# kan-bayashi/ParallelWaveGAN

Hardware: AMD Instinct MI355X
Metric: HiFi-GAN V1 22.05 kHz generator inference RTF^-1 (audio samples/s) (higher is better)
Workload: dtype f32; 1 GPU; HiFi-GAN V1 generator fwd, LJSpeech 22.05 kHz, B16 x 800 mel frames per GPU, fp32, random init; global_batch=16, parallelism=replicas x1

## Files before the change

### include/pwg_kernels.h

```cpp
#ifndef PWG_KERNELS_H_
#define PWG_KERNELS_H_

#include <stddef.h>
#include <stdint.h>

#ifdef __cplusplus
extern "C" {
#endif

typedef enum pwg_status {
  PWG_OK = 0,
  PWG_ERR_BAD_SHAPE = -1,
  PWG_ERR_UNSUPPORTED = -2,
  PWG_ERR_LAUNCH = -3,
  PWG_ERR_NULL = -4,
  PWG_ERR_WORKSPACE = -5
} pwg_status;

const char* pwg_last_error(void);
int pwg_abi_version(void);
int pwg_target_arch(void);

int pwg_prof_enable(int on);
int pwg_prof_reset(void);
// ... 64 lines not shown
int pwg_conv1d_backward_weight(const pwg_conv1d_desc* d, const float* x, const float* dy, float* dw,
                               float* db, float* workspace, size_t workspace_floats, void* stream);

size_t pwg_conv1d_backward_weight_wn_workspace_floats(const pwg_conv1d_desc* d);
int pwg_conv1d_backward_weight_wn(const pwg_conv1d_desc* d, const float* x, const float* dy, const float* v,
                                  const float* g, float* dv, float* dg, float* db, float* workspace,
                                  size_t workspace_floats, void* stream);

int pwg_conv1d_num_tile_configs(void);
int pwg_conv1d_forward_cfg(const pwg_conv1d_desc* d, const float* x, const float* w_packed,
                           const float* bias, const float* add1, const float* add2, float* y,
                           int32_t tile_config, int32_t use_dma, void* stream);

int pwg_conv1d_bf16_supported(const pwg_conv1d_desc* d);
size_t pwg_conv1d_bf16_packed_weight_bytes(const pwg_conv1d_desc* d);
int pwg_conv1d_bf16_pack_weight(const pwg_conv1d_desc* d, const float* w, const float* scale, void* w_packed,
                                void* stream);
int pwg_conv1d_bf16_forward(const pwg_conv1d_desc* d, const float* x, const void* w_packed, const float* bias,
                            const float* add1, const float* add2, float* y, float* workspace, size_t workspace_floats,
                            void* stream);
int pwg_conv1d_bf16_forward_cfg(const pwg_conv1d_desc* d, const float* x, const void* w_packed, const float* bias,
                                const float* add1, const float* add2, float* y, int32_t mfma_shape, void* stream);

int pwg_conv1d_split_supported(const pwg_conv1d_desc* d);
size_t pwg_conv1d_split_packed_weight_bytes(const pwg_conv1d_desc* d);
int pwg_conv1d_split_pack_weight(const pwg_conv1d_desc* d, const float* w, const float* scale, void* w_packed,
                                 void* stream);
int pwg_conv1d_split_forward(const pwg_conv1d_desc* d, const float* x, const void* w_packed, const float* bias,
                             const float* add1, const float* add2, float* y, float* workspace, size_t workspace_floats,
                             void* stream);
int pwg_conv1d_split_forward_cfg(const pwg_conv1d_desc* d, const float* x, const void* w_packed, const float* bias,
                                 const float* add1, const float* add2, float* y, int32_t mfma_shape, int32_t tile_mode,
                                 void* stream);

int pwg_convtr1d_split_supported(const pwg_conv1d_desc* d);
size_t pwg_convtr1d_split_packed_weight_bytes(const pwg_conv1d_desc* d);
int pwg_convtr1d_split_pack_weight(const pwg_conv1d_desc* d, const float* w, const float* scale, void* w_packed,
                                   void* stream);
int pwg_convtr1d_split_forward(const pwg_conv1d_desc* d, const float* x, const void* w_packed, const float* bias,
                               const float* add1, const float* add2, float* y, float* workspace,
                               size_t workspace_floats, void* stream);
int pwg_convtr1d_split_forward_cfg(const pwg_conv1d_desc* d, const float* x, const void* w_packed, const float* bias,
                                   const float* add1, const float* add2, float* y, int32_t mfma_shape,
                                   int32_t tile_mode, void* stream);

int pwg_conv1d_stream_supported(const pwg_conv1d_desc* d);
size_t pwg_conv1d_stream_hist_floats(const pwg_conv1d_desc* d);
int pwg_conv1d_stream_forward(const pwg_conv1d_desc* d, const float* x, const float* hist_in, float* hist_out,
                              const float* w_packed, const float* bias, const float* add1, const float* add2, float* y,
                              void* stream);

int pwg_conv1d_stream_bf16_supported(const pwg_conv1d_desc* d);
int pwg_conv1d_stream_bf16_forward(const pwg_conv1d_desc* d, const float* x, const float* hist_in, float* hist_out,
                                   const void* w_packed_bf16, const float* bias, const float* add1,
                                   const float* add2, float* y, void* stream);

int pwg_conv1d_stream_delayed_supported(const pwg_conv1d_desc* d, int32_t delay1, int32_t delay2);
int pwg_conv1d_stream_delayed_forward(const pwg_conv1d_desc* d, const float* x, const float* hist_in, float* hist_out,
                                      const float* w_packed, const float* bias, const float* add1,
                                      const float* add1_hist_in, float* add1_hist_out, int32_t delay1, const float* add2,
                                      const float* add2_hist_in, float* add2_hist_out, int32_t delay2, int32_t valid_lo,
                                      int32_t valid_hi, float* y, void* stream);

int pwg_conv1d_stream_bf16_delayed_supported(const pwg_conv1d_desc* d, int32_t delay1, int32_t delay2);
int pwg_conv1d_stream_bf16_delayed_forward(const pwg_conv1d_desc* d, const float* x, const float* hist_in,
                                           float* hist_out, const void* w_packed_bf16, const float* bias,
// ... 333 lines not shown
```

### parallelwavegan_amd/_lib.py

```python
import ctypes
import os

_HERE = os.path.dirname(os.path.abspath(__file__))
LIB_PATH = os.environ.get("PWG_KERNEL_LIB") or os.path.join(_HERE, "libpwgkernels.so")

PWG_ACT_NONE, PWG_ACT_LEAKY_RELU, PWG_ACT_TANH, PWG_ACT_RELU = 0, 1, 2, 3
PWG_PAD_ZERO, PWG_PAD_REFLECT, PWG_PAD_REPLICATE = 0, 1, 2
ABI_VERSION = 15
SPECTRAL_NORM_SCRATCH_FLOATS = 257


class ConvDesc(ctypes.Structure):

    _fields_ = [
        ("batch", ctypes.c_int32),
        ("c_in", ctypes.c_int32),
        ("c_out", ctypes.c_int32),
        ("t_in", ctypes.c_int32),
        ("t_out", ctypes.c_int32),
        ("width", ctypes.c_int32),
        ("kernel", ctypes.c_int32),
        ("stride", ctypes.c_int32),
        ("dilation", ctypes.c_int32),
        ("pad_left", ctypes.c_int32),
# ... 76 lines not shown
_i64 = ctypes.c_int64
_f32 = ctypes.c_float

SIGNATURES = {
    "pwg_last_error": (ctypes.c_char_p, []),
    "pwg_abi_version": (ctypes.c_int, []),
    "pwg_target_arch": (ctypes.c_int, []),
    "pwg_debug_poison_lds": (ctypes.c_int, [ctypes.c_int]),
    "pwg_set_concurrency_hint": (ctypes.c_float, [ctypes.c_float]),
    "pwg_prof_enable": (ctypes.c_int, [ctypes.c_int]),
    "pwg_prof_reset": (ctypes.c_int, []),
    "pwg_prof_num_kernels": (ctypes.c_int, []),
    "pwg_prof_get": (ctypes.c_int, [_i32, ctypes.c_char_p, ctypes.c_size_t, ctypes.POINTER(ctypes.c_double),
                                    ctypes.POINTER(ctypes.c_int64), ctypes.POINTER(ctypes.c_double),
                                    ctypes.POINTER(ctypes.c_double)]),
    "pwg_conv1d_packed_weight_floats": (ctypes.c_size_t, [ctypes.POINTER(ConvDesc)]),
    "pwg_conv1d_pack_weight": (ctypes.c_int, [ctypes.POINTER(ConvDesc), _vp, _vp, _vp, _vp]),
    "pwg_conv1d_forward_workspace_floats": (ctypes.c_size_t, [ctypes.POINTER(ConvDesc)]),
    "pwg_conv1d_forward": (ctypes.c_int, [ctypes.POINTER(ConvDesc), _vp, _vp, _vp, _vp, _vp, _vp, _vp, ctypes.c_size_t,
                                          _vp]),
    "pwg_conv1d_bf16_supported": (ctypes.c_int, [ctypes.POINTER(ConvDesc)]),
    "pwg_conv1d_bf16_packed_weight_bytes": (ctypes.c_size_t, [ctypes.POINTER(ConvDesc)]),
    "pwg_conv1d_bf16_pack_weight": (ctypes.c_int, [ctypes.POINTER(ConvDesc), _vp, _vp, _vp, _vp]),
    "pwg_conv1d_bf16_forward": (ctypes.c_int, [ctypes.POINTER(ConvDesc), _vp, _vp, _vp, _vp, _vp, _vp, _vp, ctypes.c_size_t,
                                               _vp]),
    "pwg_conv1d_bf16_forward_cfg": (ctypes.c_int, [ctypes.POINTER(ConvDesc), _vp, _vp, _vp, _vp, _vp, _vp, _i32, _vp]),
    "pwg_conv1d_split_supported": (ctypes.c_int, [ctypes.POINTER(ConvDesc)]),
    "pwg_conv1d_split_packed_weight_bytes": (ctypes.c_size_t, [ctypes.POINTER(ConvDesc)]),
    "pwg_conv1d_split_pack_weight": (ctypes.c_int, [ctypes.POINTER(ConvDesc), _vp, _vp, _vp, _vp]),
    "pwg_conv1d_split_forward": (ctypes.c_int, [ctypes.POINTER(ConvDesc), _vp, _vp, _vp, _vp, _vp, _vp, _vp,
                                                ctypes.c_size_t, _vp]),
    "pwg_conv1d_split_forward_cfg": (ctypes.c_int, [ctypes.POINTER(ConvDesc), _vp, _vp, _vp, _vp, _vp, _vp, _i32, _i32,
                                                    _vp]),
    "pwg_convtr1d_split_supported": (ctypes.c_int, [ctypes.POINTER(ConvDesc)]),
    "pwg_convtr1d_split_packed_weight_bytes": (ctypes.c_size_t, [ctypes.POINTER(ConvDesc)]),
    "pwg_convtr1d_split_pack_weight": (ctypes.c_int, [ctypes.POINTER(ConvDesc), _vp, _vp, _vp, _vp]),
    "pwg_convtr1d_split_forward": (ctypes.c_int, [ctypes.POINTER(ConvDesc), _vp, _vp, _vp, _vp, _vp, _vp, _vp,
                                                  ctypes.c_size_t, _vp]),
    "pwg_convtr1d_split_forward_cfg": (ctypes.c_int, [ctypes.POINTER(ConvDesc), _vp, _vp, _vp, _vp, _vp, _vp, _i32, _i32,
                                                      _vp]),
    "pwg_conv1d_stream_supported": (ctypes.c_int, [ctypes.POINTER(ConvDesc)]),
    "pwg_conv1d_stream_hist_floats": (ctypes.c_size_t, [ctypes.POINTER(ConvDesc)]),
    "pwg_conv1d_stream_forward": (ctypes.c_int, [ctypes.POINTER(ConvDesc), _vp, _vp, _vp, _vp, _vp, _vp, _vp, _vp, _vp]),
    "pwg_conv1d_stream_bf16_supported": (ctypes.c_int, [ctypes.POINTER(ConvDesc)]),
    "pwg_conv1d_stream_bf16_forward": (ctypes.c_int, [ctypes.POINTER(ConvDesc), _vp, _vp, _vp, _vp, _vp, _vp, _vp, _vp,
                                                      _vp]),
    "pwg_conv1d_stream_delayed_supported": (ctypes.c_int, [ctypes.POINTER(ConvDesc), _i32, _i32]),
    "pwg_conv1d_stream_delayed_forward": (ctypes.c_int, [ctypes.POINTER(ConvDesc), _vp, _vp, _vp, _vp, _vp, _vp, _vp, _vp,
                                                         _i32, _vp, _vp, _vp, _i32, _i32, _i32, _vp, _vp]),
    "pwg_conv1d_stream_bf16_delayed_supported": (ctypes.c_int, [ctypes.POINTER(ConvDesc), _i32, _i32]),
    "pwg_conv1d_stream_bf16_delayed_forward": (ctypes.c_int, [ctypes.POINTER(ConvDesc), _vp, _vp, _vp, _vp, _vp, _vp, _vp,
                                                              _vp, _i32, _vp, _vp, _vp, _i32, _i32, _i32, _vp, _vp]),
    "pwg_conv1d_stream_slots_forward": (ctypes.c_int, [ctypes.POINTER(ConvDesc), _vp, _vp, _vp, _vp, _vp, _vp, _vp, _vp,
                                                       _i32, _vp, _vp, _vp, _i32, _vp, _i32, _i32, _vp, _vp]),
    "pwg_conv1d_stream_slots_forward_bf16": (ctypes.c_int, [ctypes.POINTER(ConvDesc), _vp, _vp, _vp, _vp, _vp, _vp, _vp,
                                                            _vp, _i32, _vp, _vp, _vp, _i32, _vp, _i32, _i32, _vp, _vp]),
    "pwg_conv1d_stream_mirrored_supported": (ctypes.c_int, [ctypes.POINTER(ConvDesc)]),
    "pwg_conv1d_stream_mirrored_forward": (ctypes.c_int, [ctypes.POINTER(ConvDesc), _vp, _vp, _vp, _vp, _vp, _vp, _i32,
                                                          _i32, _i32, _i32, _vp]),
    "pwg_conv1d_packed_weight_bwd_floats": (ctypes.c_size_t, [ctypes.POINTER(ConvDesc)]),
    "pwg_conv1d_pack_weight_bwd": (ctypes.c_int, [ctypes.POINTER(ConvDesc), _vp, _vp, _vp, _vp]),
    "pwg_weight_bank_table_bytes": (ctypes.c_size_t, [_i32]),
    "pwg_weight_bank_build": (ctypes.c_int, [ctypes.POINTER(BankItem), _i32, _vp, ctypes.c_size_t,
                                             ctypes.POINTER(ctypes.c_int32)]),
    "pwg_weight_bank_prepare": (ctypes.c_int, [_vp, ctypes.POINTER(ctypes.c_int32), _i32, _vp]),
    "pwg_conv1d_backward_data_workspace_floats": (ctypes.c_size_t, [ctypes.POINTER(ConvDesc)]),
# ... 158 lines not shown
```

### parallelwavegan_amd/csrc/conv1d_split.hip

```cpp
#include "mfma_conv.h"

namespace pwg {
namespace {

constexpr int PARTS = 3;

struct SplitArgs : MfmaConvArgs {
  int plane;
  long part_stride;
  float pre_mul;
  unsigned pre_mask;
  int wide_out;
};

static int split_geometry(const pwg_conv1d_desc* d, MfmaConvGeom* g) {
  return mfma_conv_geometry("conv1d_split", PARTS, false, d, g);
}

__device__ __forceinline__ float pre_activate(float v, float mul, unsigned mask) {
  const float n = __uint_as_float(__float_as_uint(v * mul) & mask);
  return v > 0.f ? v : n;
}

template <int NT, bool CHECKED>
// ... 93 lines not shown
      for (int k = 0; k < NB; ++k) v[k] *= a.out_mul;
    }
    if (a.out_div != 1.0f) {
#pragma unroll
      for (int k = 0; k < NB; ++k) v[k] = v[k] / a.out_div;
    }
    if (a.post_act == PWG_ACT_LEAKY_RELU) {
#pragma unroll
      for (int k = 0; k < NB; ++k)
#pragma unroll
        for (int e = 0; e < 4; ++e) v[k][e] = v[k][e] > 0.f ? v[k][e] : v[k][e] * a.post_slope;
    } else if (a.post_act == PWG_ACT_RELU) {
#pragma unroll
      for (int k = 0; k < NB; ++k)
#pragma unroll
        for (int e = 0; e < 4; ++e) v[k][e] = v[k][e] > 0.f ? v[k][e] : 0.f;
    } else if (a.post_act == PWG_ACT_TANH) {
#pragma unroll
      for (int k = 0; k < NB; ++k) {
#pragma unroll
        for (int e = 0; e < 4; ++e) v[k][e] = tanhf(v[k][e]);
        __builtin_amdgcn_sched_barrier(0);
      }
    }
#pragma unroll
    for (int k = 0; k < NB; ++k) {
      if (WIDE) {
        if (FULL || (m < a.m && q[k] < a.nq)) *reinterpret_cast<f32x4*>(a.y + row + q[k]) = v[k];
      } else {
#pragma unroll
        for (int e = 0; e < 4; ++e)
          if (m < a.m && q[k] + e < a.nq) a.y[row + q[k] + e] = v[k][e];
      }
    }
  }
}

template <int TILE, int WM, int WN, int WAVES_M, bool VEC>
__global__ __launch_bounds__(256, WM * WN == 4 ? (TILE == 16 ? 3 : 2) : (WM * WN == 2 ? 3 : 4)) void
conv1d_split_mfma_kernel(SplitArgs a) {
  constexpr int HL = 64 / TILE;
  constexpr int KSTEPS = KC / (8 * HL);
  constexpr int TM = WM * 32 / TILE, TN = WN * 32 / TILE;
  constexpr int NREG = TILE * TILE / 64;
  constexpr int WAVES_N = 4 / WAVES_M;
  constexpr int MT = WAVES_M * WM * 32, NT = WAVES_N * WN * 32;
  typedef typename Mfma<TILE>::acc_t acc_t;

  extern __shared__ __attribute__((aligned(16))) unsigned char smem[];
  __bf16* xs = reinterpret_cast<__bf16*>(smem);

  const MfmaConvTile c = mfma_conv_tile<TILE, MT, NT, WAVES_M, VEC>(a);
  const float* __restrict__ xb = c.xb;

  acc_t acc[TM][TN];
#pragma unroll
  for (int mi = 0; mi < TM; ++mi)
#pragma unroll
    for (int ni = 0; ni < TN; ++ni)
#pragma unroll
      for (int i = 0; i < NREG; ++i) acc[mi][ni][i] = 0.f;

  for (int chunk = 0; chunk < a.cin_chunks; ++chunk) {
    if (chunk) __syncthreads();
    if (VEC) {
      const int ngroups = (c.wcols + 3) >> 2, c_left = a.c_in - chunk * KC;
// ... 19 lines not shown
            f[j] = 0.f;
            if (tin && c_base + j < a.c_in) f[j] = src[(size_t)j * a.t_in];
          }
        }
#pragma unroll
        for (int j = 0; j < 8; ++j) f[j] = pre_activate(f[j], a.pre_mul, a.pre_mask);
        split3_store<8>(f, xs + col * kConvRow + c.wave * 8, a.plane);
      }
    }
    __syncthreads();
    for (int tap = 0; tap < a.taps; ++tap) {
#pragma unroll
      for (int ks = 0; ks < KSTEPS; ++ks) {
        const int oct = ks * HL + c.h;
        const bf16x8* __restrict__ wp =
            image_rows(a.w, a.cin_chunks, a.m_pad, tap, chunk, oct) + c.m0 + c.wave_m * (WM * 32) + c.r;
        split_step<TILE, TM, TN, kConvRow, true>(wp, a.part_stride, xs, c.sh + c.wave_n * (WN * 32) + c.r + tap * a.dil,
                                                 oct * 8, a.plane, acc);
      }
    }
  }

  const size_t out_base = (size_t)c.b * a.c_out * a.t_out;
  const int row0 = c.m0 + c.wave_m * (WM * 32) + c.r, col0 = c.q0 + c.wave_n * (WN * 32) + 4 * c.h;
  const bool full = c.m0 + MT <= a.m && c.q0 + NT <= a.nq;
  if (!a.wide_out)
    split_epilogue<TILE, TM, TN, false, false>(a, acc, row0, col0, out_base);
  else if (full)
    split_epilogue<TILE, TM, TN, true, true>(a, acc, row0, col0, out_base);
  else
    split_epilogue<TILE, TM, TN, true, false>(a, acc, row0, col0, out_base);
}

template <bool VEC>
struct Family {
  template <int TILE, int WM, int WN, int WAVES_M>
  struct K {
    static constexpr auto fn = conv1d_split_mfma_kernel<TILE, WM, WN, WAVES_M, VEC>;
  };
};

static void split_fill_args(SplitArgs* a, const pwg_conv1d_desc* d, const MfmaConvGeom& g, const MfmaConvPlan& p,
                            const float* x, const void* w_packed, const float* bias, const float* add1, const float* add2,
                            float* y) {
  mfma_conv_fill_args(a, d, g, x, w_packed, bias, add1, add2, y);
  a->plane = p.plane;
  a->part_stride = image_elems(g) / 8;
  a->pre_mul = d->pre_act == PWG_ACT_LEAKY_RELU ? d->pre_slope : (d->pre_act == PWG_ACT_RELU ? 0.0f : 1.0f);
  a->pre_mask = d->pre_act == PWG_ACT_RELU ? 0u : ~0u;
  a->wide_out = d->t_out % 4 == 0 && ((reinterpret_cast<uintptr_t>(y) | reinterpret_cast<uintptr_t>(add1) |
                                       reinterpret_cast<uintptr_t>(add2)) & 15u) == 0;
}

static int split_forward(const pwg_conv1d_desc* d, const float* x, const void* w_packed, const float* bias,
                         const float* add1, const float* add2, float* y, int mfma_shape, int tile_mode,
                         hipStream_t stream) {
  MfmaConvGeom g;
  int rc = split_geometry(d, &g);
  if (rc == PWG_OK) rc = mfma_conv_check_forward("conv1d_split", d, x, w_packed, y, mfma_shape, tile_mode);
  if (rc != PWG_OK) return rc;
  const MfmaConvPlan p = mfma_conv_plan(d, g, PARTS, tile_mode, x, add1, add2);
  SplitArgs a;
  split_fill_args(&a, d, g, p, x, w_packed, bias, add1, add2, y);
  maybe_poison_lds(stream);
  ProfScope prof(stream, "conv1d_split_mfma_kernel", p.flops, p.bytes);
  if (p.vec)
    mfma_conv_launch<Family<true>::K>(p, mfma_shape, a, stream);
  else
    mfma_conv_launch<Family<false>::K>(p, mfma_shape, a, stream);
  PWG_CHECK_LAUNCH("conv1d_split");
  return PWG_OK;
}

struct ConvtrArgs : SplitArgs {
  int phases, out_off;
};

static int convtr_geometry(const pwg_conv1d_desc* d, MfmaConvGeom* g) {
  PWG_REQUIRE(d != nullptr, PWG_ERR_NULL, "convtr1d_split: NULL descriptor");
  PWG_REQUIRE(d->transposed, PWG_ERR_UNSUPPORTED,
              "convtr1d_split: not a transposed convolution (a stride-1 Conv1d runs on conv1d_split)");
  return mfma_conv_geometry("convtr1d_split", PARTS, true, d, g);
}

template <int NT, bool VEC>
__device__ __forceinline__ void stage_chunk(const SplitArgs& a, const MfmaConvTile& c, int chunk, __bf16* xs) {
  if (VEC) {
    const int ngroups = (c.wcols + 3) >> 2, c_left = a.c_in - chunk * KC;
    const float* __restrict__ xc = c.xb + (size_t)chunk * KC * a.t_in;
    if (c.base >= 0 && c.base + 4 * ngroups <= a.t_in && c_left >= KC)
      stage_window_vec<NT, false>(a, xc, c_left, c.base, ngroups, xs, c.tid);
    else
      stage_window_vec<NT, true>(a, xc, c_left, c.base, ngroups, xs, c.tid);
  } else {
    const int c_base = chunk * KC + c.wave * 8;
    const bool interior = c.base >= 0 && c.base + c.wcols <= a.t_in && c_base + 8 <= a.c_in;
    for (int col = c.lane; col < c.wcols; col += 64) {
      const int t = c.base + col;
      const float* __restrict__ src = c.xb + (size_t)c_base * a.t_in + t;
      float f[8];
      if (interior) {
#pragma unroll
        for (int j = 0; j < 8; ++j) f[j] = src[(size_t)j * a.t_in];
      } else {
        const bool tin = t >= 0 && t < a.t_in;
#pragma unroll
        for (int j = 0; j < 8; ++j) {
          f[j] = 0.f;
          if (tin && c_base + j < a.c_in) f[j] = src[(size_t)j * a.t_in];
        }
      }
#pragma unroll
      for (int j = 0; j < 8; ++j) f[j] = pre_activate(f[j], a.pre_mul, a.pre_mask);
      split3_store<8>(f, xs + col * kConvRow + c.wave * 8, a.plane);
    }
  }
}

template <int N>
__device__ __forceinline__ void convtr_finish(float out_mul, float out_div, int post_act, float post_slope, f32x4 (&v)[N],
                                              const f32x4& bias, bool has_bias, bool has1, bool has2,
                                              const f32x4 (&t1)[N], const f32x4 (&t2)[N]) {
  if (has_bias) {
#pragma unroll
    for (int k = 0; k < N; ++k) v[k] += bias;
  }
  if (has1) {
#pragma unroll
    for (int k = 0; k < N; ++k) v[k] += t1[k];
  }
  if (has2) {
#pragma unroll
    for (int k = 0; k < N; ++k) v[k] += t2[k];
  }
  if (out_mul != 1.0f) {
#pragma unroll
    for (int k = 0; k < N; ++k) v[k] *= out_mul;
  }
  if (out_div != 1.0f) {
#pragma unroll
    for (int k = 0; k < N; ++k) v[k] = v[k] / out_div;
  }
  if (post_act == PWG_ACT_LEAKY_RELU) {
#pragma unroll
    for (int k = 0; k < N; ++k)
#pragma unroll
      for (int e = 0; e < 4; ++e) v[k][e] = v[k][e] > 0.f ? v[k][e] : v[k][e] * post_slope;
  } else if (post_act == PWG_ACT_RELU) {
#pragma unroll
// ... 174 lines not shown

}
}

using namespace pwg;

extern "C" int pwg_conv1d_split_supported(const pwg_conv1d_desc* d) {
  MfmaConvGeom g;
  return split_geometry(d, &g) == PWG_OK ? 1 : 0;
}

extern "C" size_t pwg_conv1d_split_packed_weight_bytes(const pwg_conv1d_desc* d) {
  MfmaConvGeom g;
  if (split_geometry(d, &g) != PWG_OK) return 0;
  return (size_t)PARTS * image_elems(g) * sizeof(__bf16);
}

extern "C" int pwg_conv1d_split_pack_weight(const pwg_conv1d_desc* d, const float* w, const float* scale, void* w_packed,
                                            void* stream) {
  MfmaConvGeom g;
  int rc = split_geometry(d, &g);
  if (rc != PWG_OK) return rc;
  PWG_REQUIRE(w && w_packed, PWG_ERR_NULL, "conv1d_split_pack_weight: NULL pointer");
  mfma_conv_pack<PARTS>(d, g, w, scale, w_packed, (hipStream_t)stream);
  PWG_CHECK_LAUNCH("conv1d_split_pack_weight");
  return PWG_OK;
}

extern "C" int pwg_conv1d_split_forward(const pwg_conv1d_desc* d, const float* x, const void* w_packed, const float* bias,
                                        const float* add1, const float* add2, float* y, float* workspace,
                                        size_t workspace_floats, void* stream) {
  (void)workspace;
  (void)workspace_floats;
  return split_forward(d, x, w_packed, bias, add1, add2, y, kDefaultMfmaShape, 0, (hipStream_t)stream);
}

extern "C" int pwg_conv1d_split_forward_cfg(const pwg_conv1d_desc* d, const float* x, const void* w_packed,
                                            const float* bias, const float* add1, const float* add2, float* y,
                                            int32_t mfma_shape, int32_t tile_mode, void* stream) {
  return split_forward(d, x, w_packed, bias, add1, add2, y, mfma_shape, tile_mode, (hipStream_t)stream);
}

extern "C" int pwg_convtr1d_split_supported(const pwg_conv1d_desc* d) {
  MfmaConvGeom g;
  return convtr_geometry(d, &g) == PWG_OK ? 1 : 0;
}

extern "C" size_t pwg_convtr1d_split_packed_weight_bytes(const pwg_conv1d_desc* d) {
  MfmaConvGeom g;
  if (convtr_geometry(d, &g) != PWG_OK) return 0;
  return (size_t)PARTS * image_elems(g) * sizeof(__bf16);
}

extern "C" int pwg_convtr1d_split_pack_weight(const pwg_conv1d_desc* d, const float* w, const float* scale, void* w_packed,
                                              void* stream) {
  MfmaConvGeom g;
  int rc = convtr_geometry(d, &g);
  if (rc != PWG_OK) return rc;
  PWG_REQUIRE(w && w_packed, PWG_ERR_NULL, "convtr1d_split_pack_weight: NULL pointer");
  mfma_conv_pack<PARTS>(d, g, w, scale, w_packed, (hipStream_t)stream);
  PWG_CHECK_LAUNCH("convtr1d_split_pack_weight");
  return PWG_OK;
}

extern "C" int pwg_convtr1d_split_forward(const pwg_conv1d_desc* d, const float* x, const void* w_packed, const float* bias,
                                          const float* add1, const float* add2, float* y, float* workspace,
                                          size_t workspace_floats, void* stream) {
  (void)workspace;
  (void)workspace_floats;
  return convtr_forward(d, x, w_packed, bias, add1, add2, y, kDefaultMfmaShape, 0, (hipStream_t)stream);
}

extern "C" int pwg_convtr1d_split_forward_cfg(const pwg_conv1d_desc* d, const float* x, const void* w_packed,
// ... 5 lines not shown
```

### parallelwavegan_amd/csrc/resunit_split.hip

```cpp
#include "mfma_conv.h"

#include <stdlib.h>

namespace pwg {
namespace {

constexpr size_t kRuSplitMaxLds = 80 * 1024;

struct RuSplitArgs {
  const float* x;
  const bf16x8* w1;
  const float* b1;
  const bf16x8* w2;
  const float* b2;
  const float* add2;
  float* y;
  int T, k, d1;
  int bn_out;
  int hla;
  int sh;
  int p2;
  int rows;
  int plane;
  long part_stride;
  float slope1, slope2, out_div;
};

template <int C>
struct RuSplitCfg {
  static constexpr int MB = C / KC;
  static constexpr int WAVES_N = 4 / MB;
  static constexpr int H = WAVES_N * 64;
  static constexpr int ROW = C + 8;
  static constexpr int OCTS = C / 8;
  static constexpr int CHUNKS = image_chunks(C), M_PAD = image_m_pad(C);
};

template <int C, bool CHECKED>
__device__ __forceinline__ void ru_stage_window(const RuSplitArgs& a, const float* __restrict__ xb, int base, __bf16* xs,
                                                int tid) {
  constexpr int OCTS = RuSplitCfg<C>::OCTS, ROW = RuSplitCfg<C>::ROW;
  const int nitems = (a.rows >> 2) * OCTS;
  f32x4 st[2][8];
#pragma unroll
  for (int it = 0; it < 2; ++it) {
    const int idx = tid + it * 256, oct = idx % OCTS, grp = idx / OCTS;
    const int t = base + grp * 4;
    const float* __restrict__ src = xb + (size_t)(oct * 8) * a.T + t;
    const bool in = idx < nitems && (!CHECKED || (t >= 0 && t < a.T));
#pragma unroll
    for (int j = 0; j < 8; ++j) {
      f32x4 v = {0.f, 0.f, 0.f, 0.f};
      if (in) v = *reinterpret_cast<const f32x4*>(src + (size_t)j * a.T);
      st[it][j] = v;
    }
  }
#pragma unroll
  for (int it = 0; it < 2; ++it) {
    const int idx = tid + it * 256, oct = idx % OCTS, grp = idx / OCTS;
    if (idx < nitems) {
#pragma unroll
      for (int e = 0; e < 4; ++e) {
        float v[8];
#pragma unroll
        for (int j = 0; j < 8; ++j) {
          const float s = st[it][j][e];
          v[j] = s > 0.f ? s : s * a.slope1;
        }
        split3_store<8>(v, xs + (grp * 4 + e) * ROW + oct * 8, a.plane);
        __builtin_amdgcn_sched_barrier(0);
      }
    }
  }
}

template <int C, int TILE>
__device__ __forceinline__ void ru_request(bf16x8 (&wf)[3], const bf16x8* __restrict__ w, long part_stride, unsigned wrow,
                                           int h) {
  using Cfg = RuSplitCfg<C>;
  split_step_request(wf, w, part_stride, wrow + split_step_rows<TILE>(Cfg::CHUNKS, Cfg::M_PAD, SplitStepId{0, 0, 0}, h));
}
template <int C, int TILE, bool XFIRST>
__device__ __forceinline__ void ru_contract(bf16x8 (&wf)[3], const bf16x8* __restrict__ w, long part_stride, unsigned wrow,
                                            const __bf16* bl, int plane, int tap_step, int taps, int h,
                                            typename Mfma<TILE>::acc_t (&acc)[32 / TILE][64 / TILE]) {
  using Cfg = RuSplitCfg<C>;
  constexpr int HL = 64 / TILE, KSTEPS = KC / (8 * HL), TM = 32 / TILE, TN = 64 / TILE;
  SplitStepId step{0, 0, 0};
#pragma unroll 1
  for (int s = 0; s < Cfg::CHUNKS * taps * KSTEPS; ++s) {
    const SplitStepId next = split_step_successor(step, Cfg::CHUNKS, taps, KSTEPS);
    split_step_streamed<TILE, TM, TN, Cfg::ROW, XFIRST>(
        wf, w, part_stride, wrow + split_step_rows<TILE>(Cfg::CHUNKS, Cfg::M_PAD, step, h),
        wrow + split_step_rows<TILE>(Cfg::CHUNKS, Cfg::M_PAD, next, h), bl, step.tap * tap_step,
        step.chunk * KC + split_step_off<TILE>(step, h), plane, acc);
    step = next;
  }
}

template <int C, int TILE>
__global__ __launch_bounds__(256, 2) void resunit_split_kernel(RuSplitArgs a) {
  using Cfg = RuSplitCfg<C>;
  constexpr int WAVES_N = Cfg::WAVES_N, ROW = Cfg::ROW, H = Cfg::H;
  constexpr int HL = 64 / TILE, TM = 32 / TILE, TN = 64 / TILE, NREG = TILE * TILE / 64, NG = NREG / 4;
  typedef typename Mfma<TILE>::acc_t acc_t;
  extern __shared__ __attribute__((aligned(16))) unsigned char smem[];
  __bf16* xs = reinterpret_cast<__bf16*>(smem);

  const int tid = threadIdx.x, lane = tid & 63;
  const int wave = __builtin_amdgcn_readfirstlane(tid >> 6);
  const int wave_m = wave / WAVES_N, wave_n = wave % WAVES_N;
  const int r = lane & (TILE - 1), h = lane / TILE;
  const int b = blockIdx.y;
  const int t0 = blockIdx.x * a.bn_out;
  const int base = t0 - a.hla;
  const int T = a.T;
  const bool pair = a.w2 != nullptr;
  const float* __restrict__ xb = a.x + (size_t)b * C * T;

  const unsigned wrow = wave_m * 32 + r;
  bf16x8 wf[3];
  ru_request<C, TILE>(wf, a.w1, a.part_stride, wrow, h);

  if (base >= 0 && base + a.rows <= T)
    ru_stage_window<C, false>(a, xb, base, xs, tid);
  else
    ru_stage_window<C, true>(a, xb, base, xs, tid);

  acc_t acc[TM][TN];
#pragma unroll
  for (int mi = 0; mi < TM; ++mi)
#pragma unroll
    for (int ni = 0; ni < TN; ++ni)
#pragma unroll
      for (int i = 0; i < NREG; ++i) acc[mi][ni][i] = 0.f;
  __syncthreads();

  if (pair) {
    ru_contract<C, TILE, false>(wf, a.w1, a.part_stride, wrow, xs + (wave_n * 64 + r + a.sh) * ROW, a.plane, a.d1, a.k,
                                h, acc);
    ru_request<C, TILE>(wf, a.w2, a.part_stride, wrow, h);
    __syncthreads();
    const bool has_b1 = a.b1 != nullptr;
#pragma unroll
    for (int mi = 0; mi < TM; ++mi)
#pragma unroll
      for (int g = 0; g < NG; ++g) {
        const int c = wave_m * 32 + mi * TILE + 4 * h + 4 * HL * g;
        f32x4 bias = {0.f, 0.f, 0.f, 0.f};
        if (has_b1) {
#pragma unroll
          for (int e = 0; e < 4; ++e) bias[e] = a.b1[c + e];
        }
#pragma unroll
        for (int ni = 0; ni < TN; ++ni) {
          const int m = wave_n * 64 + ni * TILE + r;
          const int th = t0 - a.p2 + m;
          const bool inside = th >= 0 && th < T;
          float v[4];
#pragma unroll
          for (int e = 0; e < 4; ++e) {
            v[e] = acc[mi][ni][4 * g + e];
            if (has_b1) v[e] += bias[e];
            v[e] = v[e] > 0.f ? v[e] : v[e] * a.slope2;
            v[e] = inside ? v[e] : 0.f;
            acc[mi][ni][4 * g + e] = 0.f;
          }
          split3_store<4>(v, xs + m * ROW + c, a.plane);
        }
      }
    for (int i = tid; i < (a.k - 1) * Cfg::OCTS; i += 256) {
      bf16x8 z;
#pragma unroll
      for (int j = 0; j < 8; ++j) z[j] = (__bf16)0.f;
      __bf16* dst = xs + (H + i / Cfg::OCTS) * ROW + (i % Cfg::OCTS) * 8;
      *reinterpret_cast<bf16x8*>(dst) = z;
      *reinterpret_cast<bf16x8*>(dst + a.plane) = z;
      *reinterpret_cast<bf16x8*>(dst + 2 * a.plane) = z;
    }
    __syncthreads();
    ru_contract<C, TILE, true>(wf, a.w2, a.part_stride, wrow, xs + (wave_n * 64 + r) * ROW, a.plane, 1, a.k, h,
                               acc);
  } else {
    ru_contract<C, TILE, true>(wf, a.w1, a.part_stride, wrow, xs + (wave_n * 64 + r + a.sh) * ROW, a.plane, a.d1, a.k,
                               h, acc);
  }

  constexpr int NV = TN * NG;
  const float* __restrict__ bias_p = pair ? a.b2 : a.b1;
  const bool has_bias = bias_p != nullptr, has2 = a.add2 != nullptr;
#pragma unroll
  for (int mi = 0; mi < TM; ++mi) {
    const int c = wave_m * 32 + mi * TILE + r;
    const size_t row = ((size_t)b * C + c) * T;
    int t[NV];
    bool ok[NV];
#pragma unroll
    for (int n = 0; n < NV; ++n) {
      const int slot = wave_n * 64 + (n / NG) * TILE + 4 * h + 4 * HL * (n % NG);
      ok[n] = slot < a.bn_out && t0 + slot < T;
      t[n] = ok[n] ? t0 + slot : t0;
    }
    f32x4 t1[NV], t2[NV], v[NV];
    float bias = 0.f;
    if (has_bias) bias = bias_p[c];
#pragma unroll
    for (int n = 0; n < NV; ++n) t1[n] = *reinterpret_cast<const f32x4*>(a.x + row + t[n]);
    if (has2) {
#pragma unroll
      for (int n = 0; n < NV; ++n) t2[n] = *reinterpret_cast<const f32x4*>(a.add2 + row + t[n]);
    }
#pragma unroll
    for (int n = 0; n < NV; ++n)
#pragma unroll
      for (int e = 0; e < 4; ++e) v[n][e] = acc[mi][n / NG][(n % NG) * 4 + e];
    if (has_bias) {
#pragma unroll
      for (int n = 0; n < NV; ++n) v[n] += bias;
    }
#pragma unroll
    for (int n = 0; n < NV; ++n) v[n] += t1[n];
    if (has2) {
#pragma unroll
      for (int n = 0; n < NV; ++n) v[n] += t2[n];
    }
    if (a.out_div != 1.0f) {
#pragma unroll
      for (int n = 0; n < NV; ++n) v[n] = v[n] / a.out_div;
    }
#pragma unroll
    for (int n = 0; n < NV; ++n)
      if (ok[n]) *reinterpret_cast<f32x4*>(a.y + row + t[n]) = v[n];
  }
}

struct RuSplitGeom {
  int hla, sh, p2, bn_out, rows, tiles;
  size_t lds;
};

static int ru_split_geometry(const pwg_resunit_desc* d, RuSplitGeom* g) {
  PWG_REQUIRE(d != nullptr, PWG_ERR_NULL, "resunit_split: NULL descriptor");
  const int C = d->channels;
  PWG_REQUIRE(C == 32 || C == 64, PWG_ERR_UNSUPPORTED, "resunit_split: channels = %d (only 32 and 64)", C);
// ... 102 lines not shown
```

### parallelwavegan_amd/ops.py

```python
import ctypes

import torch

from . import _lib
from ._lib import ConvDesc, ResUnitDesc, WaveNetDesc

ACT = {None: _lib.PWG_ACT_NONE, "none": _lib.PWG_ACT_NONE, "leaky_relu": _lib.PWG_ACT_LEAKY_RELU,
       "tanh": _lib.PWG_ACT_TANH, "relu": _lib.PWG_ACT_RELU}
PAD = {"zero": _lib.PWG_PAD_ZERO, "reflect": _lib.PWG_PAD_REFLECT, "replicate": _lib.PWG_PAD_REPLICATE}


PARAM_EPOCH = [0]


def bump_param_epoch():
    PARAM_EPOCH[0] += 1


def cache_epoch():
    return PARAM_EPOCH[0]


def param_epoch(p):
    return getattr(p, "_pwg_epoch", 0)
# ... 132 lines not shown
    if out is None:
        out = torch.empty((desc.batch, desc.c_out, desc.t_out * desc.width), device=x.device, dtype=torch.float32)
    assert x.numel() == desc.batch * desc.c_in * desc.t_in * desc.width, (tuple(x.shape), desc.batch, desc.c_in, desc.t_in)
    assert out.numel() == desc.batch * desc.c_out * desc.t_out * desc.width
    ws, ws_n = _workspace(_lib.lib().pwg_conv1d_forward_workspace_floats(ctypes.byref(desc)), x.device)
    _lib.check(_lib.lib().pwg_conv1d_forward(ctypes.byref(desc), _ptr(x), _ptr(w_packed), _ptr(bias), _ptr(add1),
                                             _ptr(add2), _ptr(out), _ptr(ws), ws_n, _stream()), "conv1d_forward")
    return out


def conv1d_bf16_supported(desc):
    return bool(_lib.lib().pwg_conv1d_bf16_supported(ctypes.byref(desc)))


def _zero_padded(desc):
    if desc.pad_mode == PAD["zero"]:
        return desc
    desc = ConvDesc.from_buffer_copy(desc)
    desc.pad_mode = PAD["zero"]
    return desc


def _pack_weight_mfma(kind, desc, w, scale, op="conv1d"):
    _require_device(w, scale)
    n = getattr(_lib.lib(), f"pwg_{op}_{kind}_packed_weight_bytes")(ctypes.byref(desc))
    if n == 0:
        _lib.check(-1, f"{op}_{kind}_packed_weight_bytes")
    out = torch.empty(n, device=w.device, dtype=torch.uint8)
    pack = getattr(_lib.lib(), f"pwg_{op}_{kind}_pack_weight")
    _lib.check(pack(ctypes.byref(desc), _ptr(w), _ptr(scale), _ptr(out), _stream()), f"{op}_{kind}_pack_weight")
    return out


def _conv1d_forward_mfma(kind, desc, image_desc, x, w_packed, bias, add1, add2, out, cfg, op="conv1d"):
    name = f"{op}_forward_{kind}"
    _require_device(x, bias, add1, add2, out)
    if not w_packed.is_cuda or w_packed.dtype != torch.uint8:
        raise RuntimeError(f"{name}: w_packed must be the device image of pack_weight_{kind}")
    if out is None:
        out = torch.empty((desc.batch, desc.c_out, desc.t_out), device=x.device, dtype=torch.float32)
    assert x.numel() == desc.batch * desc.c_in * desc.t_in, (tuple(x.shape), desc.batch, desc.c_in, desc.t_in)
    assert out.numel() == desc.batch * desc.c_out * desc.t_out
    image_bytes = getattr(_lib.lib(), f"pwg_{op}_{kind}_packed_weight_bytes")(ctypes.byref(image_desc))
    if image_bytes == 0:
        _lib.check(-1, f"{op}_{kind}_packed_weight_bytes")
    assert w_packed.numel() == image_bytes, f"{name}: w_packed is not this layer's {kind} image"
    for t in (add1, add2):
        assert t is None or t.numel() == out.numel()
    args = (ctypes.byref(desc), _ptr(x), _ptr(w_packed), _ptr(bias), _ptr(add1), _ptr(add2), _ptr(out))
    if cfg is None:
        rc = getattr(_lib.lib(), f"pwg_{op}_{kind}_forward")(*args, None, 0, _stream())
    else:
        rc = getattr(_lib.lib(), f"pwg_{op}_{kind}_forward_cfg")(*args, *cfg, _stream())
    _lib.check(rc, name)
    return out


def pack_weight_bf16(desc, w, scale=None):
    return _pack_weight_mfma("bf16", _zero_padded(desc), w, scale)


def conv1d_forward_bf16(desc, x, w_packed, bias=None, add1=None, add2=None, out=None, mfma_shape=None):
    return _conv1d_forward_mfma("bf16", desc, _zero_padded(desc), x, w_packed, bias, add1, add2, out,
                                None if mfma_shape is None else (int(mfma_shape),))


def conv1d_split_supported(desc):
    return bool(_lib.lib().pwg_conv1d_split_supported(ctypes.byref(desc)))


def pack_weight_split(desc, w, scale=None):
    return _pack_weight_mfma("split", desc, w, scale)


def conv1d_forward_split(desc, x, w_packed, bias=None, add1=None, add2=None, out=None, mfma_shape=None, tile_mode=0):
    cfg = None if mfma_shape is None and not tile_mode else (int(mfma_shape or 16), int(tile_mode))
    return _conv1d_forward_mfma("split", desc, desc, x, w_packed, bias, add1, add2, out, cfg)


def convtr1d_split_supported(desc):
    return bool(_lib.lib().pwg_convtr1d_split_supported(ctypes.byref(desc)))


def pack_weight_split_transposed(desc, w, scale=None):
    return _pack_weight_mfma("split", desc, w, scale, op="convtr1d")


def conv1d_forward_split_transposed(desc, x, w_packed, bias=None, add1=None, add2=None, out=None, mfma_shape=None,
                                    tile_mode=0):
    cfg = None if mfma_shape is None and not tile_mode else (int(mfma_shape or 16), int(tile_mode))
    return _conv1d_forward_mfma("split", desc, desc, x, w_packed, bias, add1, add2, out, cfg, op="convtr1d")


def conv1d_stream_supported(desc):
    return bool(_lib.lib().pwg_conv1d_stream_supported(ctypes.byref(desc)))


def conv1d_stream_hist_floats(desc):
    return _lib.lib().pwg_conv1d_stream_hist_floats(ctypes.byref(desc))


def _conv1d_stream_out(desc, x, hist_in, hist_out, add1, add2, out):
    if out is None:
        out = torch.empty((desc.batch, desc.c_out, desc.t_out), device=x.device, dtype=torch.float32)
    assert x.numel() == desc.batch * desc.c_in * desc.t_in, (tuple(x.shape), desc.batch, desc.c_in, desc.t_in)
    assert out.numel() == desc.batch * desc.c_out * desc.t_out
    n_hist = conv1d_stream_hist_floats(desc)
    for t in (hist_in, hist_out):
# ... 679 lines not shown
```

Before: 77.85 million samples/s.

## Add streamed-weight step kernel for split conv1d; prefetch resunit epilogue operands

Adds a streamed variant of the split-bf16 MFMA conv1d kernel. It double-buffers weight fragments across taps and K-steps, fetching the next step's weights while the current step computes. A plan heuristic selects it for layers with at least 7 taps and 2 or more input chunks. Separately, the residual-unit kernel now issues loads for the residual, add2 and bias values during window staging and the first contraction, so their latency is hidden before the epilogue. The cost is more live registers for the prefetched operands, which may lower occupancy.

```diff
diff --git a/include/pwg_kernels.h b/include/pwg_kernels.h
--- a/include/pwg_kernels.h
+++ b/include/pwg_kernels.h
@@ -120,6 +120,10 @@
 int pwg_conv1d_split_forward_cfg(const pwg_conv1d_desc* d, const float* x, const void* w_packed, const float* bias,
                                  const float* add1, const float* add2, float* y, int32_t mfma_shape, int32_t tile_mode,
                                  void* stream);
+int pwg_conv1d_split_step_form(const pwg_conv1d_desc* d);
+int pwg_conv1d_split_forward_step(const pwg_conv1d_desc* d, const float* x, const void* w_packed, const float* bias,
+                                  const float* add1, const float* add2, float* y, int32_t mfma_shape, int32_t tile_mode,
+                                  int32_t step_form, void* stream);
 
 int pwg_convtr1d_split_supported(const pwg_conv1d_desc* d);
 size_t pwg_convtr1d_split_packed_weight_bytes(const pwg_conv1d_desc* d);
diff --git a/parallelwavegan_amd/_lib.py b/parallelwavegan_amd/_lib.py
--- a/parallelwavegan_amd/_lib.py
+++ b/parallelwavegan_amd/_lib.py
@@ -132,6 +132,9 @@
                                                 ctypes.c_size_t, _vp]),
     "pwg_conv1d_split_forward_cfg": (ctypes.c_int, [ctypes.POINTER(ConvDesc), _vp, _vp, _vp, _vp, _vp, _vp, _i32, _i32,
                                                     _vp]),
+    "pwg_conv1d_split_step_form": (ctypes.c_int, [ctypes.POINTER(ConvDesc)]),
+    "pwg_conv1d_split_forward_step": (ctypes.c_int, [ctypes.POINTER(ConvDesc), _vp, _vp, _vp, _vp, _vp, _vp, _i32, _i32,
+                                                     _i32, _vp]),
     "pwg_convtr1d_split_supported": (ctypes.c_int, [ctypes.POINTER(ConvDesc)]),
     "pwg_convtr1d_split_packed_weight_bytes": (ctypes.c_size_t, [ctypes.POINTER(ConvDesc)]),
     "pwg_convtr1d_split_pack_weight": (ctypes.c_int, [ctypes.POINTER(ConvDesc), _vp, _vp, _vp, _vp]),
diff --git a/parallelwavegan_amd/csrc/conv1d_split.hip b/parallelwavegan_amd/csrc/conv1d_split.hip
--- a/parallelwavegan_amd/csrc/conv1d_split.hip
+++ b/parallelwavegan_amd/csrc/conv1d_split.hip
@@ -149,6 +149,40 @@
         for (int e = 0; e < 4; ++e)
           if (m < a.m && q[k] + e < a.nq) a.y[row + q[k] + e] = v[k][e];
       }
+    }
+  }
+}
+
+template <int NT, bool VEC>
+__device__ __forceinline__ void stage_chunk(const SplitArgs& a, const MfmaConvTile& c, int chunk, __bf16* xs) {
+  if (VEC) {
+    const int ngroups = (c.wcols + 3) >> 2, c_left = a.c_in - chunk * KC;
+    const float* __restrict__ xc = c.xb + (size_t)chunk * KC * a.t_in;
+    if (c.base >= 0 && c.base + 4 * ngroups <= a.t_in && c_left >= KC)
+      stage_window_vec<NT, false>(a, xc, c_left, c.base, ngroups, xs, c.tid);
+    else
+      stage_window_vec<NT, true>(a, xc, c_left, c.base, ngroups, xs, c.tid);
+  } else {
+    const int c_base = chunk * KC + c.wave * 8;
+    const bool interior = c.base >= 0 && c.base + c.wcols <= a.t_in && c_base + 8 <= a.c_in;
+    for (int col = c.lane; col < c.wcols; col += 64) {
+      const int t = c.base + col;
+      const float* __restrict__ src = c.xb + (size_t)c_base * a.t_in + t;
+      float f[8];
+      if (interior) {
+#pragma unroll
+        for (int j = 0; j < 8; ++j) f[j] = src[(size_t)j * a.t_in];
+      } else {
+        const bool tin = t >= 0 && t < a.t_in;
+#pragma unroll
+        for (int j = 0; j < 8; ++j) {
+          f[j] = 0.f;
+          if (tin && c_base + j < a.c_in) f[j] = src[(size_t)j * a.t_in];
+        }
+      }
+#pragma unroll
+      for (int j = 0; j < 8; ++j) f[j] = pre_activate(f[j], a.pre_mul, a.pre_mask);
+      split3_store<8>(f, xs + col * kConvRow + c.wave * 8, a.plane);
     }
   }
 }
@@ -234,11 +268,67 @@
     split_epilogue<TILE, TM, TN, true, false>(a, acc, row0, col0, out_base);
 }
 
-template <bool VEC>
+template <int TILE, int WM, int WN, int WAVES_M, bool VEC>
+__global__ __launch_bounds__(256, WM * WN == 4 ? (TILE == 16 ? 3 : 2) : (WM * WN == 2 ? 3 : 4)) void
+conv1d_split_streamed_mfma_kernel(SplitArgs a) {
+  constexpr int HL = 64 / TILE;
+  constexpr int KSTEPS = KC / (8 * HL);
+  constexpr int TM = WM * 32 / TILE, TN = WN * 32 / TILE;
+  constexpr int NREG = TILE * TILE / 64;
+  constexpr int WAVES_N = 4 / WAVES_M;
+  constexpr int MT = WAVES_M * WM * 32, NT = WAVES_N * WN * 32;
+  typedef typename Mfma<TILE>::acc_t acc_t;
+
+  extern __shared__ __attribute__((aligned(16))) unsigned char smem[];
+  __bf16* xs = reinterpret_cast<__bf16*>(smem);
+
+  const MfmaConvTile c = mfma_conv_tile<TILE, MT, NT, WAVES_M, VEC>(a);
+
+  const unsigned wrow = c.m0 + c.wave_m * (WM * 32) + c.r;
+  bf16x8 wf[3];
+  SplitStepId step{0, 0, 0};
+  split_step_request(wf, a.w, a.part_stride, wrow + split_step_rows<TILE>(a.cin_chunks, a.m_pad, step, c.h));
+
+  acc_t acc[TM][TN];
+#pragma unroll
+  for (int mi = 0; mi < TM; ++mi)
+#pragma unroll
+    for (int ni = 0; ni < TN; ++ni)
+#pragma unroll
+      for (int i = 0; i < NREG; ++i) acc[mi][ni][i] = 0.f;
+
+  for (int chunk = 0; chunk < a.cin_chunks; ++chunk) {
+    if (chunk) __syncthreads();
+    stage_chunk<NT, VEC>(a, c, chunk, xs);
+    __syncthreads();
+#pragma unroll 1
+    for (int s = 0; s < a.taps * KSTEPS; ++s) {
+      const SplitStepId next = split_step_successor(step, a.cin_chunks, a.taps, KSTEPS);
+      split_step_streamed<TILE, TM, TN, kConvRow, true>(
+          wf, a.w, a.part_stride, wrow + split_step_rows<TILE>(a.cin_chunks, a.m_pad, step, c.h),
+          wrow + split_step_rows<TILE>(a.cin_chunks, a.m_pad, next, c.h), xs,
+          c.sh + c.wave_n * (WN * 32) + c.r + step.tap * a.dil, split_step_off<TILE>(step, c.h), a.plane, acc);
+      step = next;
+    }
+  }
+
+  const size_t out_base = (size_t)c.b * a.c_out * a.t_out;
+  const int row0 = c.m0 + c.wave_m * (WM * 32) + c.r, col0 = c.q0 + c.wave_n * (WN * 32) + 4 * c.h;
+  const bool full = c.m0 + MT <= a.m && c.q0 + NT <= a.nq;
+  if (!a.wide_out)
+    split_epilogue<TILE, TM, TN, false, false>(a, acc, row0, col0, out_base);
+  else if (full)
+    split_epilogue<TILE, TM, TN, true, true>(a, acc, row0, col0, out_base);
+  else
+    split_epilogue<TILE, TM, TN, true, false>(a, acc, row0, col0, out_base);
+}
+
+template <bool VEC, bool STREAMED>
 struct Family {
   template <int TILE, int WM, int WN, int WAVES_M>
   struct K {
-    static constexpr auto fn = conv1d_split_mfma_kernel<TILE, WM, WN, WAVES_M, VEC>;
+    static constexpr auto fn = STREAMED ? conv1d_split_streamed_mfma_kernel<TILE, WM, WN, WAVES_M, VEC>
+                                        : conv1d_split_mfma_kernel<TILE, WM, WN, WAVES_M, VEC>;
   };
 };
 
@@ -254,22 +344,42 @@
                                        reinterpret_cast<uintptr_t>(add2)) & 15u) == 0;
 }
 
+constexpr int kStepPlanDecides = 0, kStepResident = 1, kStepStreamed = 2;
+constexpr int kStreamedMinTaps = 7, kStreamedMinChunks = 2;
+static int split_step_form(const MfmaConvGeom& g) {
+  if (!split_image_addressable(image_elems(g))) return kStepResident;
+  return g.taps >= kStreamedMinTaps && g.cin_chunks >= kStreamedMinChunks ? kStepStreamed : kStepResident;
+}
+
 static int split_forward(const pwg_conv1d_desc* d, const float* x, const void* w_packed, const float* bias,
-                         const float* add1, const float* add2, float* y, int mfma_shape, int tile_mode,
+                         const float* add1, const float* add2, float* y, int mfma_shape, int tile_mode, int step_form,
                          hipStream_t stream) {
   MfmaConvGeom g;
   int rc = split_geometry(d, &g);
-  if (rc == PWG_OK) rc = mfma_conv_check_forward("conv1d_split", d, x, w_packed, y, mfma_shape, tile_mode);
+  if (rc != PWG_OK) return rc;
+  PWG_REQUIRE(step_form >= kStepPlanDecides && step_form <= kStepStreamed, PWG_ERR_BAD_SHAPE,
+              "conv1d_split: step_form = %d (0 = the plan decides, 1 = resident, 2 = streamed)", step_form);
+  rc = mfma_conv_check_forward("conv1d_split", d, x, w_packed, y, mfma_shape, tile_mode);
   if (rc != PWG_OK) return rc;
   const MfmaConvPlan p = mfma_conv_plan(d, g, PARTS, tile_mode, x, add1, add2);
+  PWG_REQUIRE(step_form != kStepStreamed || split_image_addressable(image_elems(g)), PWG_ERR_UNSUPPORTED,
+              "conv1d_split: weight image too large for the streamed step");
+  const bool streamed = (step_form == kStepPlanDecides ? split_step_form(g) : step_form) == kStepStreamed;
   SplitArgs a;
   split_fill_args(&a, d, g, p, x, w_packed, bias, add1, add2, y);
   maybe_poison_lds(stream);
   ProfScope prof(stream, "conv1d_split_mfma_kernel", p.flops, p.bytes);
-  if (p.vec)
-    mfma_conv_launch<Family<true>::K>(p, mfma_shape, a, stream);
-  else
-    mfma_conv_launch<Family<false>::K>(p, mfma_shape, a, stream);
+  if (p.vec) {
+    if (streamed)
+      mfma_conv_launch<Family<true, true>::K>(p, mfma_shape, a, stream);
+    else
+      mfma_conv_launch<Family<true, false>::K>(p, mfma_shape, a, stream);
+  } else {
+    if (streamed)
+      mfma_conv_launch<Family<false, true>::K>(p, mfma_shape, a, stream);
+    else
+      mfma_conv_launch<Family<false, false>::K>(p, mfma_shape, a, stream);
+  }
   PWG_CHECK_LAUNCH("conv1d_split");
   return PWG_OK;
 }
@@ -283,40 +393,6 @@
   PWG_REQUIRE(d->transposed, PWG_ERR_UNSUPPORTED,
               "convtr1d_split: not a transposed convolution (a stride-1 Conv1d runs on conv1d_split)");
   return mfma_conv_geometry("convtr1d_split", PARTS, true, d, g);
-}
-
-template <int NT, bool VEC>
-__device__ __forceinline__ void stage_chunk(const SplitArgs& a, const MfmaConvTile& c, int chunk, __bf16* xs) {
-  if (VEC) {
-    const int ngroups = (c.wcols + 3) >> 2, c_left = a.c_in - chunk * KC;
-    const float* __restrict__ xc = c.xb + (size_t)chunk * KC * a.t_in;
-    if (c.base >= 0 && c.base + 4 * ngroups <= a.t_in && c_left >= KC)
-      stage_window_vec<NT, false>(a, xc, c_left, c.base, ngroups, xs, c.tid);
-    else
-      stage_window_vec<NT, true>(a, xc, c_left, c.base, ngroups, xs, c.tid);
-  } else {
-    const int c_base = chunk * KC + c.wave * 8;
-    const bool interior = c.base >= 0 && c.base + c.wcols <= a.t_in && c_base + 8 <= a.c_in;
-    for (int col = c.lane; col < c.wcols; col += 64) {
-      const int t = c.base + col;
-      const float* __restrict__ src = c.xb + (size_t)c_base * a.t_in + t;
-      float f[8];
-      if (interior) {
-#pragma unroll
-        for (int j = 0; j < 8; ++j) f[j] = src[(size_t)j * a.t_in];
-      } else {
-        const bool tin = t >= 0 && t < a.t_in;
-#pragma unroll
-        for (int j = 0; j < 8; ++j) {
-          f[j] = 0.f;
-          if (tin && c_base + j < a.c_in) f[j] = src[(size_t)j * a.t_in];
-        }
-      }
-#pragma unroll
-      for (int j = 0; j < 8; ++j) f[j] = pre_activate(f[j], a.pre_mul, a.pre_mask);
-      split3_store<8>(f, xs + col * kConvRow + c.wave * 8, a.plane);
-    }
-  }
 }
 
 template <int N>
@@ -557,13 +633,25 @@
                                         size_t workspace_floats, void* stream) {
   (void)workspace;
   (void)workspace_floats;
-  return split_forward(d, x, w_packed, bias, add1, add2, y, kDefaultMfmaShape, 0, (hipStream_t)stream);
+  return split_forward(d, x, w_packed, bias, add1, add2, y, kDefaultMfmaShape, 0, kStepPlanDecides, (hipStream_t)stream);
 }
 
 extern "C" int pwg_conv1d_split_forward_cfg(const pwg_conv1d_desc* d, const float* x, const void* w_packed,
                                             const float* bias, const float* add1, const float* add2, float* y,
                                             int32_t mfma_shape, int32_t tile_mode, void* stream) {
-  return split_forward(d, x, w_packed, bias, add1, add2, y, mfma_shape, tile_mode, (hipStream_t)stream);
+  return split_forward(d, x, w_packed, bias, add1, add2, y, mfma_shape, tile_mode, kStepPlanDecides, (hipStream_t)stream);
+}
+
+extern "C" int pwg_conv1d_split_forward_step(const pwg_conv1d_desc* d, const float* x, const void* w_packed,
+                                             const float* bias, const float* add1, const float* add2, float* y,
+                                             int32_t mfma_shape, int32_t tile_mode, int32_t step_form, void* stream) {
+  return split_forward(d, x, w_packed, bias, add1, add2, y, mfma_shape, tile_mode, step_form, (hipStream_t)stream);
+}
+
+extern "C" int pwg_conv1d_split_step_form(const pwg_conv1d_desc* d) {
+  MfmaConvGeom g;
+  if (split_geometry(d, &g) != PWG_OK) return 0;
+  return split_step_form(g);
 }
 
 extern "C" int pwg_convtr1d_split_supported(const pwg_conv1d_desc* d) {
diff --git a/parallelwavegan_amd/csrc/resunit_split.hip b/parallelwavegan_amd/csrc/resunit_split.hip
--- a/parallelwavegan_amd/csrc/resunit_split.hip
+++ b/parallelwavegan_amd/csrc/resunit_split.hip
@@ -36,9 +36,9 @@
   static constexpr int CHUNKS = image_chunks(C), M_PAD = image_m_pad(C);
 };
 
-template <int C, bool CHECKED>
+template <int C, bool CHECKED, typename Behind>
 __device__ __forceinline__ void ru_stage_window(const RuSplitArgs& a, const float* __restrict__ xb, int base, __bf16* xs,
-                                                int tid) {
+                                                int tid, Behind&& behind) {
   constexpr int OCTS = RuSplitCfg<C>::OCTS, ROW = RuSplitCfg<C>::ROW;
   const int nitems = (a.rows >> 2) * OCTS;
   f32x4 st[2][8];
@@ -55,6 +55,7 @@
       st[it][j] = v;
     }
   }
+  behind();
 #pragma unroll
   for (int it = 0; it < 2; ++it) {
     const int idx = tid + it * 256, oct = idx % OCTS, grp = idx / OCTS;
@@ -98,6 +99,12 @@
   }
 }
 
+template <int TILE>
+__device__ __forceinline__ int ru_out_slot(int wave_n, int h, int n) {
+  constexpr int HL = 64 / TILE, NG = TILE * TILE / 256;
+  return wave_n * 64 + (n / NG) * TILE + 4 * h + 4 * HL * (n % NG);
+}
+
 template <int C, int TILE>
 __global__ __launch_bounds__(256, 2) void resunit_split_kernel(RuSplitArgs a) {
   using Cfg = RuSplitCfg<C>;
@@ -122,10 +129,56 @@
   bf16x8 wf[3];
   ru_request<C, TILE>(wf, a.w1, a.part_stride, wrow, h);
 
+  constexpr int NV = TN * NG;
+  const bool has2 = a.add2 != nullptr;
+  f32x4 res[TM][NV], ad2[TM][NV];
+  auto request_values = [&](const float* __restrict__ src, f32x4 (&dst)[TM][NV]) {
+    __builtin_amdgcn_sched_barrier(0);
+#pragma unroll
+    for (int mi = 0; mi < TM; ++mi) {
+      const float* __restrict__ rowp = src + ((size_t)b * C + wave_m * 32 + mi * TILE + r) * T;
+#pragma unroll
+      for (int n = 0; n < NV; ++n) {
+        const int slot = ru_out_slot<TILE>(wave_n, h, n);
+        const bool ok = slot < a.bn_out && t0 + slot < T;
+        dst[mi][n] = *reinterpret_cast<const f32x4*>(rowp + (ok ? t0 + slot : t0));
+      }
+    }
+    __builtin_amdgcn_sched_barrier(0);
+  };
+#pragma unroll
+  for (int mi = 0; mi < TM; ++mi)
+#pragma unroll
+    for (int n = 0; n < NV; ++n) ad2[mi][n] = f32x4{0.f, 0.f, 0.f, 0.f};
+  const float* __restrict__ bias_p = pair ? a.b2 : a.b1;
+  const bool has_b1 = a.b1 != nullptr, has_bias = bias_p != nullptr;
+  f32x4 bias_h[TM][NG];
+  float bias_y[TM];
+#pragma unroll
+  for (int mi = 0; mi < TM; ++mi) {
+    bias_y[mi] = 0.f;
+#pragma unroll
+    for (int g = 0; g < NG; ++g) bias_h[mi][g] = f32x4{0.f, 0.f, 0.f, 0.f};
+  }
+  auto behind_window = [&] {
+    request_values(a.x, res);
+    if (!pair && has2) request_values(a.add2, ad2);
+#pragma unroll
+    for (int mi = 0; mi < TM; ++mi) {
+      if (has_bias) bias_y[mi] = bias_p[wave_m * 32 + mi * TILE + r];
+      if (pair && has_b1) {
+#pragma unroll
+        for (int g = 0; g < NG; ++g)
+#pragma unroll
+          for (int e = 0; e < 4; ++e) bias_h[mi][g][e] = a.b1[wave_m * 32 + mi * TILE + 4 * h + 4 * HL * g + e];
+      }
+    }
+    __builtin_amdgcn_sched_barrier(0);
+  };
   if (base >= 0 && base + a.rows <= T)
-    ru_stage_window<C, false>(a, xb, base, xs, tid);
+    ru_stage_window<C, false>(a, xb, base, xs, tid, behind_window);
   else
-    ru_stage_window<C, true>(a, xb, base, xs, tid);
+    ru_stage_window<C, true>(a, xb, base, xs, tid, behind_window);
 
   acc_t acc[TM][TN];
 #pragma unroll
@@ -140,18 +193,14 @@
     ru_contract<C, TILE, false>(wf, a.w1, a.part_stride, wrow, xs + (wave_n * 64 + r + a.sh) * ROW, a.plane, a.d1, a.k,
                                 h, acc);
     ru_request<C, TILE>(wf, a.w2, a.part_stride, wrow, h);
+    if (has2) request_values(a.add2, ad2);
     __syncthreads();
-    const bool has_b1 = a.b1 != nullptr;
 #pragma unroll
     for (int mi = 0; mi < TM; ++mi)
 #pragma unroll
       for (int g = 0; g < NG; ++g) {
         const int c = wave_m * 32 + mi * TILE + 4 * h + 4 * HL * g;
-        f32x4 bias = {0.f, 0.f, 0.f, 0.f};
-        if (has_b1) {
-#pragma unroll
-          for (int e = 0; e < 4; ++e) bias[e] = a.b1[c + e];
-        }
+        const f32x4 bias = bias_h[mi][g];
 #pragma unroll
         for (int ni = 0; ni < TN; ++ni) {
           const int m = wave_n * 64 + ni * TILE + r;
@@ -186,9 +235,6 @@
                                h, acc);
   }
 
-  constexpr int NV = TN * NG;
-  const float* __restrict__ bias_p = pair ? a.b2 : a.b1;
-  const bool has_bias = bias_p != nullptr, has2 = a.add2 != nullptr;
 #pragma unroll
   for (int mi = 0; mi < TM; ++mi) {
     const int c = wave_m * 32 + mi * TILE + r;
@@ -197,19 +243,14 @@
     bool ok[NV];
 #pragma unroll
     for (int n = 0; n < NV; ++n) {
-      const int slot = wave_n * 64 + (n / NG) * TILE + 4 * h + 4 * HL * (n % NG);
+      const int slot = ru_out_slot<TILE>(wave_n, h, n);
       ok[n] = slot < a.bn_out && t0 + slot < T;
       t[n] = ok[n] ? t0 + slot : t0;
     }
-    f32x4 t1[NV], t2[NV], v[NV];
-    float bias = 0.f;
-    if (has_bias) bias = bias_p[c];
-#pragma unroll
-    for (int n = 0; n < NV; ++n) t1[n] = *reinterpret_cast<const f32x4*>(a.x + row + t[n]);
-    if (has2) {
-#pragma unroll
-      for (int n = 0; n < NV; ++n) t2[n] = *reinterpret_cast<const f32x4*>(a.add2 + row + t[n]);
-    }
+    const f32x4(&t1)[NV] = res[mi];
+    const f32x4(&t2)[NV] = ad2[mi];
+    f32x4 v[NV];
+    const float bias = bias_y[mi];
 #pragma unroll
     for (int n = 0; n < NV; ++n)
 #pragma unroll
diff --git a/parallelwavegan_amd/ops.py b/parallelwavegan_amd/ops.py
--- a/parallelwavegan_amd/ops.py
+++ b/parallelwavegan_amd/ops.py
@@ -188,7 +188,7 @@
     return out
 
 
-def _conv1d_forward_mfma(kind, desc, image_desc, x, w_packed, bias, add1, add2, out, cfg, op="conv1d"):
+def _conv1d_forward_mfma(kind, desc, image_desc, x, w_packed, bias, add1, add2, out, cfg, op="conv1d", entry="cfg"):
     name = f"{op}_forward_{kind}"
     _require_device(x, bias, add1, add2, out)
     if not w_packed.is_cuda or w_packed.dtype != torch.uint8:
@@ -207,7 +207,7 @@
     if cfg is None:
         rc = getattr(_lib.lib(), f"pwg_{op}_{kind}_forward")(*args, None, 0, _stream())
     else:
-        rc = getattr(_lib.lib(), f"pwg_{op}_{kind}_forward_cfg")(*args, *cfg, _stream())
+        rc = getattr(_lib.lib(), f"pwg_{op}_{kind}_forward_{entry}")(*args, *cfg, _stream())
     _lib.check(rc, name)
     return out
 
@@ -229,7 +229,21 @@
     return _pack_weight_mfma("split", desc, w, scale)
 
 
-def conv1d_forward_split(desc, x, w_packed, bias=None, add1=None, add2=None, out=None, mfma_shape=None, tile_mode=0):
+STEP_FORMS = {1: "resident", 2: "streamed"}
+
+
+def conv1d_split_step_form(desc):
+    form = _lib.lib().pwg_conv1d_split_step_form(ctypes.byref(desc))
+    if form == 0:
+        _lib.check(-1, "conv1d_split_step_form")
+    return STEP_FORMS[form]
+
+
+def conv1d_forward_split(desc, x, w_packed, bias=None, add1=None, add2=None, out=None, mfma_shape=None, tile_mode=0,
+                         step_form=0):
+    if step_form:
+        cfg = (int(mfma_shape or 16), int(tile_mode), int(step_form))
+        return _conv1d_forward_mfma("split", desc, desc, x, w_packed, bias, add1, add2, out, cfg, entry="step")
     cfg = None if mfma_shape is None and not tile_mode else (int(mfma_shape or 16), int(tile_mode))
     return _conv1d_forward_mfma("split", desc, desc, x, w_packed, bias, add1, add2, out, cfg)
 
```

Result: faster. 79.87 million samples/s, median of 6 (+2.6%).
